# vita-epfl/trajnetplusplusbaselines

Measured on NVIDIA H100. Metric: pedestrian-steps/sec, higher is better.
Workload: dtype f32

## Files before the change

trajnetplusplusbaselines_b200/csrc/capi.cu:

```cuda
#include <algorithm>
#include <cstdio>
#include <cstdlib>
#include <cstring>
#include <new>

#include "common.cuh"

namespace tb2 {

static thread_local std::string g_error;
std::atomic<uint64_t> g_launch_count{0};

void set_error(const std::string& msg) { g_error = msg; }

struct ProfRec { const char* name; cudaEvent_t a, b; };
static bool g_profiling = false;
static std::vector<ProfRec> g_prof;

KernelTimer::KernelTimer(const char* name, cudaStream_t s) : slot(-1), st(s) {
    if (!g_profiling) return;
    ProfRec r;
    r.name = name;
    if (cudaEventCreate(&r.a) != cudaSuccess || cudaEventCreate(&r.b) != cudaSuccess) return;
    cudaEventRecord(r.a, st);
// ... 211 lines not shown
                TB2_REQUIRE(m->mlp_dims[i] >= 1, "MLP width");
            }
            m->pool_out = m->n_mlp == 0 ? m->mlp_dims[0] : c.out_dim;
            break;
        case TB2_POOL_NN_LSTM:
            TB2_REQUIRE(c.mlp_dim_hidden >= 1 && c.mlp_dim_hidden <= 512 && c.out_dim <= 1024 && c.mlp_dim_vel != 0,
                        "nearest-neighbour LSTM pooling needs 1 <= hidden_dim <= 512, out_dim <= 1024 and velocities");
            [[fallthrough]];
        case TB2_POOL_NN_MLP:
            TB2_REQUIRE(c.n >= 1 && c.n <= 32 && c.mlp_dim_spatial >= 1 && c.out_dim == c.n * c.mlp_dim_spatial,
                        "nearest-neighbour pooling needs 1 <= n <= 32 and out_dim == n * mlp_dim_spatial");
            m->pool_out = c.out_dim;
            break;
        case TB2_POOL_TRAJECTRON:
            TB2_REQUIRE(c.mlp_dim_hidden >= 1 && c.mlp_dim_hidden <= 512 && c.out_dim >= 1 && c.out_dim <= 1024,
                        "Trajectron pooling needs 1 <= hidden_dim <= 512 and out_dim <= 1024");
            m->pool_out = c.out_dim;
            break;
        case TB2_POOL_ATTN_MLP:
            TB2_REQUIRE(c.mlp_dim_spatial >= 1 && c.mlp_dim_vel >= 0 && c.mlp_dim_hidden >= 0 && c.out_dim >= 1 &&
                            c.mlp_dim_spatial + c.mlp_dim_vel + c.mlp_dim_hidden <= 128,
                        "attention pooling needs mlp_dim <= 128 (kernel specialisation)");
            m->pool_out = c.out_dim;
            break;
        case TB2_POOL_HIDDEN_MLP:
            TB2_REQUIRE(c.mlp_dim_spatial >= 1 && c.mlp_dim_vel >= 0 && c.mlp_dim_hidden >= 0 && c.out_dim >= 1 &&
                            c.mlp_dim_spatial + c.mlp_dim_vel + c.mlp_dim_hidden <= 4096,
                        "hidden-state MLP pooling widths");
            m->pool_out = c.out_dim;
            break;
    }
    TB2_REQUIRE(c.pool_to_input || m->pool_out == m->H, "pool_to_input=0 needs out_dim == hidden_dim");
    m->P = c.pool_to_input ? m->pool_out : 0;
    return TB2_OK;
}

static int alloc_buffers(tb2_lstm* m) {
    const tb2_lstm_config& c = m->cfg;
    int rc;
#define ALLOC(ptr, count) if ((rc = dev_alloc(m->owned, (void**)&(ptr), (size_t)(count) * sizeof(float)))) return rc
    ALLOC(m->We, (m->E - 2) * 2);
    ALLOC(m->be, m->E - 2);
    ALLOC(m->Wn, 5 * m->H);
    ALLOC(m->bn, 5);
    for (int ph = 0; ph < 2; ++ph) {
        ALLOC(m->WgT[ph], (size_t)m->K_gate_pad * 4 * m->H);
        ALLOC(m->bg[ph], 4 * m->H);
    }
    const bool no_tc = m->tc_disabled;
    if (!no_tc && gates_tc_supported(m)) {
        const size_t half = ((size_t)4 * m->H * m->K_gate + 1) / 2;
        for (int ph = 0; ph < 2; ++ph) {
            float *hi, *lo;
            ALLOC(hi, half);
            ALLOC(lo, half);
            m->Wg_hi[ph] = hi;
            m->Wg_lo[ph] = lo;
        }
    }
    const size_t Hp = (size_t)c.mlp_dim_hidden, D = (size_t)(c.mlp_dim_spatial + c.mlp_dim_vel + c.mlp_dim_hidden);
    auto encoder_lstm = [&]() {
        ALLOC(m->pl_WihT, (size_t)c.out_dim * 4 * Hp);
        ALLOC(m->pl_WhhT, Hp * 4 * Hp);
        ALLOC(m->pl_b, 4 * Hp);
        ALLOC(m->mp_WoT, Hp * (size_t)c.out_dim);
        ALLOC(m->mp_bo, c.out_dim);
        return TB2_OK;
    };
    switch (c.pool_type) {
        case TB2_POOL_NONE:
            break;
        case TB2_POOL_SOCIAL:
            ALLOC(m->WencT, m->H * m->C);
            ALLOC(m->benc, m->C);
            [[fallthrough]];
        case TB2_POOL_OCCUPANCY:
        case TB2_POOL_DIRECTIONAL:
            if (m->n_mlp == 0) break;
            ALLOC(m->Wt1, (size_t)m->cells * m->C * m->mlp_dims[1]);
            ALLOC(m->base1, m->mlp_dims[1]);
            if (c.pool_type == TB2_POOL_SOCIAL && m->C == 16 && !no_tc) {
                const size_t half = ((size_t)m->cells * 16 * m->mlp_dims[1] + 1) / 2;
                float *hi, *lo;
                ALLOC(hi, 2 * half);
                ALLOC(lo, 4);
                m->Wt1_hi = hi;
                m->Wt1_lo = lo;
            }
            for (int layer = 1; layer < m->n_mlp; ++layer) {
                ALLOC(m->WT[layer], (size_t)m->mlp_dims[layer] * m->mlp_dims[layer + 1]);
                ALLOC(m->bl[layer], m->mlp_dims[layer + 1]);
                if (layer == 1 && !no_tc && dense_tc_supported(m->mlp_dims[1], m->mlp_dims[2])) {
                    const size_t half = ((size_t)m->mlp_dims[1] * m->mlp_dims[2] + 1) / 2;
                    float *hi, *lo;
                    ALLOC(hi, half);
                    ALLOC(lo, half);
                    m->W_hi[1] = hi;
                    m->W_lo[1] = lo;
                }
            }
            break;
        case TB2_POOL_NN_LSTM:
            if ((rc = encoder_lstm())) return rc;
            [[fallthrough]];
        case TB2_POOL_NN_MLP:
            ALLOC(m->mp_Ws, c.mlp_dim_spatial * 4);
            ALLOC(m->mp_bs, c.mlp_dim_spatial);
            break;
        case TB2_POOL_TRAJECTRON:
            ALLOC(m->mp_Ws, (size_t)c.out_dim * 8);
            ALLOC(m->mp_bs, c.out_dim);
            if ((rc = encoder_lstm())) return rc;
            break;
        case TB2_POOL_ATTN_MLP:
            ALLOC(m->at_AqT, D * D);
            ALLOC(m->at_Ak, D * D);
            ALLOC(m->at_AvT, D * D);
            ALLOC(m->at_bqkv, 3 * D);
            ALLOC(m->at_WoT, D * D);
            ALLOC(m->at_bo, D);
            [[fallthrough]];
        case TB2_POOL_HIDDEN_MLP:
            ALLOC(m->mp_Ws, c.mlp_dim_spatial * 2);
            ALLOC(m->mp_bs, c.mlp_dim_spatial);
            ALLOC(m->mp_Wv, std::max(c.mlp_dim_vel, 1) * 2);
            ALLOC(m->mp_bv, std::max(c.mlp_dim_vel, 1));
            ALLOC(m->mp_WhT, (size_t)m->H * std::max(c.mlp_dim_hidden, 1));
            ALLOC(m->mp_bh, std::max(c.mlp_dim_hidden, 1));
            ALLOC(m->mp_WoT, D * c.out_dim);
            ALLOC(m->mp_bo, c.out_dim);
            break;
    }
#undef ALLOC
    return TB2_OK;
}

int tb2_lstm_create(const tb2_lstm_config* cfg, tb2_lstm** out) {
    TB2_REQUIRE(cfg && out, "null argument");
    *out = nullptr;
    if (!hidden_dim_supported(cfg->hidden_dim)) {
        set_error(kHiddenDimMessage);
        return TB2_ERR_UNSUPPORTED;
    }
    TB2_REQUIRE(cfg->embedding_dim >= 4 && cfg->embedding_dim <= 1024, "embedding_dim out of range");
    TB2_REQUIRE(cfg->pool_type >= TB2_POOL_NONE && cfg->pool_type <= TB2_POOL_TRAJECTRON, "bad pool_type");
    tb2_lstm* m = new (std::nothrow) tb2_lstm();
    TB2_REQUIRE(m, "out of host memory");
    m->cfg = *cfg;
    m->H = cfg->hidden_dim;
    m->E = cfg->embedding_dim;
    m->tc_disabled = tensor_cores_disabled();
    int rc = configure_pool(*cfg, m);
    if (rc == TB2_OK) {
        m->K_gate = m->E + m->P + m->H;
        m->K_gate_pad = (m->K_gate + kGateBK - 1) / kGateBK * kGateBK;
        rc = alloc_buffers(m);
    }
    if (rc != TB2_OK) {
        tb2_lstm_destroy(m);
        return rc;
    }
    *out = m;
    return TB2_OK;
}

int tb2_lstm_destroy(tb2_lstm* m) {
    if (!m) return TB2_OK;
// ... 336 lines not shown
```

trajnetplusplusbaselines_b200/csrc/common.cuh:

```cuda
#pragma once
#include <cuda_runtime.h>
#include <stdint.h>
#include <stddef.h>
#include <atomic>
#include <string>
#include <vector>

#include "trajnet_b200.h"

namespace tb2 {

void set_error(const std::string& msg);
extern std::atomic<uint64_t> g_launch_count;

#define TB2_CHECK_CUDA(expr)                                                              \
    do {                                                                                  \
        cudaError_t _e = (expr);                                                          \
        if (_e != cudaSuccess) {                                                          \
            ::tb2::set_error(std::string(#expr) + ": " + cudaGetErrorString(_e));         \
            return TB2_ERR_CUDA;                                                          \
        }                                                                                 \
    } while (0)

#define TB2_REQUIRE(cond, msg)                                                            \
// ... 7 lines not shown
#define TB2_LAUNCH_CHECK()                                                                \
    do {                                                                                  \
        ::tb2::g_launch_count.fetch_add(1, std::memory_order_relaxed);                    \
        TB2_CHECK_CUDA(cudaGetLastError());                                               \
    } while (0)

#ifdef __CUDACC__
__device__ __forceinline__ void grid_dep_wait() { asm volatile("griddepcontrol.wait;" ::: "memory"); }
__device__ __forceinline__ void grid_dep_launch() { asm volatile("griddepcontrol.launch_dependents;" ::: "memory"); }

__device__ __forceinline__ void mma_bf16_16816(float (&d)[4], const uint32_t (&a)[4], uint32_t b0, uint32_t b1) {
    asm volatile(
        "mma.sync.aligned.m16n8k16.row.col.f32.bf16.bf16.f32 {%0, %1, %2, %3}, {%4, %5, %6, %7}, {%8, %9}, "
        "{%0, %1, %2, %3};"
        : "+f"(d[0]), "+f"(d[1]), "+f"(d[2]), "+f"(d[3])
        : "r"(a[0]), "r"(a[1]), "r"(a[2]), "r"(a[3]), "r"(b0), "r"(b1));
}

template <typename... KArgs, typename... Args>
inline cudaError_t launch_pdl(void (*kernel)(KArgs...), dim3 grid, dim3 block, size_t smem, cudaStream_t st,
                              Args&&... args) {
    cudaLaunchConfig_t cfg = {};
    cfg.gridDim = grid;
    cfg.blockDim = block;
    cfg.dynamicSmemBytes = smem;
    cfg.stream = st;
    cudaLaunchAttribute attr[1];
    attr[0].id = cudaLaunchAttributeProgrammaticStreamSerialization;
    attr[0].val.programmaticStreamSerializationAllowed = 1;
    cfg.attrs = attr;
    cfg.numAttrs = 1;
    return cudaLaunchKernelEx(&cfg, kernel, static_cast<KArgs>(args)...);
}

template <typename... KArgs, typename... Args>
inline cudaError_t launch_pdl_cluster(void (*kernel)(KArgs...), dim3 grid, dim3 block, size_t smem, cudaStream_t st,
                                      unsigned cluster_x, Args&&... args) {
    cudaLaunchConfig_t cfg = {};
    cfg.gridDim = grid;
    cfg.blockDim = block;
    cfg.dynamicSmemBytes = smem;
    cfg.stream = st;
    cudaLaunchAttribute attr[2];
    attr[0].id = cudaLaunchAttributeProgrammaticStreamSerialization;
    attr[0].val.programmaticStreamSerializationAllowed = 1;
    attr[1].id = cudaLaunchAttributeClusterDimension;
    attr[1].val.clusterDim.x = cluster_x;
    attr[1].val.clusterDim.y = 1;
    attr[1].val.clusterDim.z = 1;
    cfg.attrs = attr;
    cfg.numAttrs = 2;
    return cudaLaunchKernelEx(&cfg, kernel, static_cast<KArgs>(args)...);
}
#endif

struct DynSmemConfig {
    size_t bytes[64];
    template <typename K>
    cudaError_t ensure(K kernel, size_t smem, size_t preset = 0) {
        int dev = 0;
        cudaError_t e = cudaGetDevice(&dev);
        if (e != cudaSuccess) return e;
        size_t& have = bytes[dev & 63];
        if (have < preset) have = preset;
        if (smem <= have) return cudaSuccess;
        e = cudaFuncSetAttribute(kernel, cudaFuncAttributeMaxDynamicSharedMemorySize, (int)smem);
        if (e == cudaSuccess) have = smem;
        return e;
    }
};

struct KernelTimer {
    KernelTimer(const char* name, cudaStream_t st);
    ~KernelTimer();
    int slot;
    cudaStream_t st;
};

constexpr int kMaxMlpLayers = 3;
constexpr int kMaxHidden = 256;
inline bool hidden_dim_supported(int H) { return H >= 32 && H <= kMaxHidden && H % 32 == 0; }
constexpr const char* kHiddenDimMessage = "hidden_dim must be a multiple of 32 from 32 to 256 (32, 64, 96, ..., 256)";
constexpr int kGateBK = 16;

}

struct tb2_lstm {
    tb2_lstm_config cfg = {};
    int H = 0, E = 0, C = 0, cells = 0, n_mlp = 0;
    int P = 0;
    int pool_out = 0;
    int mlp_dims[tb2::kMaxMlpLayers + 1] = {};
    int K_gate = 0, K_gate_pad = 0;
    bool weights_set = false;
    bool tc_disabled = false;
    float* We = nullptr;
    float* be = nullptr;
    float* WgT[2] = {};
    float* bg[2] = {};
    float* Wn = nullptr;
    float* bn = nullptr;
    float* WencT = nullptr;
    float* benc = nullptr;
    float* Wt1 = nullptr;
    float* base1 = nullptr;
    void* Wt1_hi = nullptr;
    void* Wt1_lo = nullptr;
    float* WT[tb2::kMaxMlpLayers] = {};
    float* bl[tb2::kMaxMlpLayers] = {};
    void* W_hi[tb2::kMaxMlpLayers] = {};
    void* W_lo[tb2::kMaxMlpLayers] = {};
    std::vector<cudaEvent_t> step_events;
    float *mp_Ws = nullptr, *mp_bs = nullptr, *mp_Wv = nullptr, *mp_bv = nullptr, *mp_WhT = nullptr, *mp_bh = nullptr,
          *mp_WoT = nullptr, *mp_bo = nullptr;
    float *at_AqT = nullptr, *at_Ak = nullptr, *at_AvT = nullptr, *at_bqkv = nullptr, *at_WoT = nullptr, *at_bo = nullptr;
    float *pl_WihT = nullptr, *pl_WhhT = nullptr, *pl_b = nullptr;
    void* Wg_hi[2] = {};
    void* Wg_lo[2] = {};
    std::vector<void*> owned;
};

struct tb2_layout {
    int B, M, n_max;
    int pad_to_max = 1;
    std::vector<int> scene_off_host;
    int* scene_off;
    int* row_scene;
    int group_cap[2];
    int num_groups[2];
    int* group_off[2];
    std::vector<void*> owned;
};

namespace tb2 {

struct Workspace {
    float* obs1;
    float* obs2;
    float* lat;
    int* win_count;
    uint32_t* win_ent;
    float* win_val;
    int* pair_cell;
    uint8_t* pair_flag;
    float* act[2];
    float* act2;
    float* pooled;
    void* emb_hi;
    void* emb_lo;
    void* pool_hi;
    void* pool_lo;
    void* hs_hi[2];
    void* hs_lo[2];
    size_t bytes;
    int write_pairs;
    float* pool_feat;
    float* pool_h;
    float* pool_c;
    float* scene_sum;
};

struct TrainCache {
    float* lat;
    int* win_count;
    uint32_t* win_ent;
    int* pair_cell;
// ... 50 lines not shown
```

trajnetplusplusbaselines_b200/csrc/pool.cu:

```cuda
#include <cuda_bf16.h>
#include <math_constants.h>
#include <algorithm>

#include "common.cuh"

namespace tb2 {

__global__ void resolve_obs_kernel(const float2* __restrict__ base, const float2* __restrict__ pred,
                                   const int* __restrict__ row_scene,
                                   const int* __restrict__ scene_off, float2* __restrict__ out, int M) {
    grid_dep_wait();
    grid_dep_launch();
    int m = blockIdx.x * blockDim.x + threadIdx.x;
    if (m >= M) return;
    bool primary = (scene_off[row_scene[m]] == m);
    out[m] = primary ? pred[m] : base[m];
}

int launch_resolve_obs(const tb2_layout* l, const float* base, const float* pred, float* out,
                       cudaStream_t st) {
    int threads = 256, blocks = (l->M + threads - 1) / threads;
    {
        KernelTimer kt("resolve_obs", st);
        launch_pdl(resolve_obs_kernel, dim3(blocks), dim3(threads), 0, st, (const float2*)base, (const float2*)pred,
                   (const int*)l->row_scene, (const int*)l->scene_off, (float2*)out, l->M);
    }
    TB2_LAUNCH_CHECK();
    return TB2_OK;
}

constexpr int kPrepMaxThreads = 640;
static int prep_threads(int n_max) { return 32 * std::min(std::max(n_max, 8), kPrepMaxThreads / 32); }
constexpr int kMaxSceneForPrep = 256;

struct PrepParams {
    const float2* obs1;
    const float2* obs2;
    const float* hidden;
    const int* scene_off;
    const float* WencT;
    const float* benc;
    float* lat;
    int* win_count;
    uint32_t* win_ent;
    float* win_val;
    int* pair_cell;
    uint8_t* pair_flag;
    const float* We;
    const float* be;
    __nv_bfloat16* emb_hi;
    __nv_bfloat16* emb_lo;
    int E;
    int n_max, H, C, n, pool_type, front, skip_masked, write_pairs, pad_to_max;
    float side, width;
};

__device__ __forceinline__ void cp_async16(void* smem, const void* gmem) {
    asm volatile("cp.async.cg.shared.global [%0], [%1], 16;" ::"r"((uint32_t)__cvta_generic_to_shared(smem)), "l"(gmem) : "memory");
}
__device__ __forceinline__ void cp_async_commit() { asm volatile("cp.async.commit_group;" ::: "memory"); }
__device__ __forceinline__ void cp_async_wait_all() { asm volatile("cp.async.wait_group 0;" ::: "memory"); }

__device__ __forceinline__ float nan_to_num_f(float x) {
    if (isnan(x)) return 0.f;
    if (isinf(x)) return x > 0 ? 3.402823466e+38f : -3.402823466e+38f;
    return x;
}

__global__ void __launch_bounds__(kPrepMaxThreads, 2) pool_prepare_kernel(PrepParams p) {
    const int kPrepThreads = (int)blockDim.x, kPrepWarps = kPrepThreads >> 5;
    extern __shared__ __align__(16) float smem_prep[];
    const int scene = blockIdx.x;
    const int row0 = p.scene_off[scene];
    const int n_s = p.scene_off[scene + 1] - row0;
    const int nm1 = p.n_max - 1;
    float2* pos = reinterpret_cast<float2*>(smem_prep);
    float2* vel = pos + n_s;
    int* cellrow = reinterpret_cast<int*>(vel + n_s);
    float* Ws = reinterpret_cast<float*>(cellrow + ((kPrepWarps * (nm1 > 0 ? nm1 : 1) + 3) & ~3));
    float* hs = Ws + (p.H + 8) * p.C;
    const int tid = threadIdx.x, lane = tid & 31, warp = tid >> 5;
    const bool social = p.pool_type == TB2_POOL_SOCIAL;
    const bool fast_lat = social && p.C == 16 && p.H == 128;
    if (fast_lat) {
        for (int idx = tid; idx < 128 * 4; idx += kPrepThreads) {
            const int k = idx >> 2, q4 = idx & 3;
            cp_async16(Ws + (k >> 4) * 272 + (k & 15) * 16 + q4 * 4, p.WencT + k * 16 + q4 * 4);
        }
    } else if (social) {
        for (int idx = tid; idx < p.H * p.C; idx += kPrepThreads) {
            const int k = idx / p.C, c = idx - k * p.C;
            Ws[c * (p.H + 4) + k] = p.WencT[idx];
        }
    }
    grid_dep_wait();
    grid_dep_launch();

    if (fast_lat) {
        const float* hsrc = p.hidden + (size_t)row0 * 128;
        for (int idx = tid; idx < n_s * 32; idx += kPrepThreads) cp_async16(hs + idx * 4, hsrc + idx * 4);
    }
    cp_async_commit();
    for (int j = tid; j < n_s; j += kPrepThreads) {
        float2 a = p.obs1[row0 + j], b = p.obs2[row0 + j];
        vel[j] = make_float2(b.x - a.x, b.y - a.y);
        if (isnan(b.x) || isnan(b.y)) b = make_float2(-500.f, -500.f);
        pos[j] = b;
    }
    if (social && !fast_lat) {
        const float4* hsrc = reinterpret_cast<const float4*>(p.hidden + (size_t)row0 * p.H);
        float4* hdst = reinterpret_cast<float4*>(hs);
        for (int idx = tid; idx < n_s * p.H / 4; idx += kPrepThreads) {
            float4 v = hsrc[idx];
            v.x = nan_to_num_f(v.x); v.y = nan_to_num_f(v.y); v.z = nan_to_num_f(v.z); v.w = nan_to_num_f(v.w);
            hdst[idx] = v;
        }
    }
    cp_async_wait_all();
    __syncthreads();
    if (p.emb_hi != nullptr) {
        const int e_shift = (p.E & (p.E - 1)) == 0 ? 31 - __clz(p.E) : -1;
        for (int idx = tid; idx < n_s * p.E; idx += kPrepThreads) {
            const int j = e_shift >= 0 ? idx >> e_shift : idx / p.E, k = idx - j * p.E;
            const float2 v = vel[j];
            float e = 0.f;
            if (k < p.E - 2 && !isnan(v.x))
                e = fmaxf(fmaf(p.We[2 * k + 1], v.y * 4.0f, fmaf(p.We[2 * k], v.x * 4.0f, p.be[k])), 0.f);
            const __nv_bfloat16 h = __float2bfloat16_rn(e);
            p.emb_hi[(size_t)(row0 + j) * p.E + k] = h;
            p.emb_lo[(size_t)(row0 + j) * p.E + k] = __float2bfloat16_rn(e - __bfloat162float(h));
        }
    }
    if (fast_lat) {
        const int c4 = lane & 3, kq = lane >> 2;
        const float4* wp = reinterpret_cast<const float4*>(Ws + kq * 272) + c4;
        const float4 bc = *reinterpret_cast<const float4*>(p.benc + c4 * 4);
        for (int j = warp; j < n_s; j += kPrepWarps) {
            const float4* hp = reinterpret_cast<const float4*>(hs + j * 128 + kq * 16);
            float4 acc = make_float4(0.f, 0.f, 0.f, 0.f);
#pragma unroll
            for (int q = 0; q < 4; ++q) {
// ... 284 lines not shown
        int incl = sum;
        for (int d = 1; d < 32; d <<= 1) {
            int v = __shfl_up_sync(0xffffffffu, incl, d);
            if (tid >= d) incl += v;
        }
        int run = incl - sum;
        for (int c = lo; c < hi; ++c) {
            int cnt = cursor[c];
            start[c] = run;
            cursor[c] = run;
            run += cnt;
        }
        if (tid == 31) start[bins] = incl;
    }
    __syncthreads();
    for (int idx = tid; idx < total; idx += kL1Threads) {
        int r = idx / p.nm1, k = idx - r * p.nm1;
        if (k < cnt_s[r]) {
            size_t g = (size_t)(row0 + r) * p.nm1 + k;
            uint32_t ent = raw[idx];
            int pos = atomicAdd(&cursor[(ent >> 16) * 2 + (r & 1)], 1);
            entP[pos] = (uint16_t)r;
            if (SOCIAL) {
                const int j = (int)(ent & 0xffff);
                entS[pos] = (uint16_t)(j == 0xffff ? p.cap : sbase[r] + j);
            } else {
#pragma unroll
                for (int c = 0; c < C; ++c) entV[(size_t)pos * C + c] = p.win_val[g * 2 + c] - p.constant;
            }
        }
    }
    __syncthreads();

    float w[C], wn[C];
    const float* wcol = p.Wt + col;
#pragma unroll
    for (int c = 0; c < C; ++c) w[c] = col_ok ? wcol[(size_t)c * p.OUT] : 0.f;
    for (int cell = 0; cell < p.cells; ++cell) {
        if (cell + 1 < p.cells) {
#pragma unroll
            for (int c = 0; c < C; ++c)
                wn[c] = col_ok ? wcol[((size_t)(cell + 1) * C + c) * p.OUT] : 0.f;
        }
        const int e0 = start[cell * 2 + half], e1 = start[cell * 2 + half + 1];
        for (int e = e0; e < e1; ++e) {
            const int r = entP[e];
            float a = acc[r * kL1Cols + colc];
            if (SOCIAL) {
                const float4* lv = reinterpret_cast<const float4*>(latS + (size_t)entS[e] * C);
#pragma unroll
                for (int c4 = 0; c4 < C / 4; ++c4) {
                    float4 v = lv[c4];
                    a = fmaf(v.x, w[c4 * 4 + 0], a);
                    a = fmaf(v.y, w[c4 * 4 + 1], a);
                    a = fmaf(v.z, w[c4 * 4 + 2], a);
                    a = fmaf(v.w, w[c4 * 4 + 3], a);
                }
            } else {
#pragma unroll
                for (int c = 0; c < C; ++c) a = fmaf(entV[(size_t)e * C + c], w[c], a);
            }
            acc[r * kL1Cols + colc] = a;
        }
#pragma unroll
        for (int c = 0; c < C; ++c) w[c] = wn[c];
    }
    __syncthreads();
    if (col_ok) {
        for (int r = half; r < P; r += 2) {
            float v = acc[r * kL1Cols + colc];
            if (p.relu) v = fmaxf(v, 0.f);
            const size_t o = (size_t)(row0 + r) * p.OUT + col;
            if (p.out_hi) {
                const __nv_bfloat16 h = __float2bfloat16_rn(v);
                p.out_hi[o] = h;
                p.out_lo[o] = __float2bfloat16_rn(v - __bfloat162float(h));
            } else {
                p.out[o] = v;
            }
        }
    }
}

constexpr int kMmaAccStride = kL1Cols + 16;

#ifndef TB2_L1_ABLATE
#define TB2_L1_ABLATE 0
#endif

__device__ __forceinline__ int kperm16(int k) { return 4 * ((k & 7) >> 1) + 2 * (k >> 3) + (k & 1); }

struct L1MmaParams {
    const int* group_off;
    const int* scene_off;
    const int* win_count;
    const uint32_t* win_ent;
    const float* lat;
    const float* benc;
    const __nv_bfloat16* Wt_hi;
    const __nv_bfloat16* Wt_lo;
    const float* base;
    float* out;
    __nv_bfloat16* out_hi;
    __nv_bfloat16* out_lo;
    int OUT, cells, nm1, cap, relu;
    float constant;
};

constexpr int kMmaThreads = 512;
constexpr int kMmaDepth = 8;
constexpr int kMmaMaxCap = 254;

__host__ __device__ inline size_t l1_mma_max_tiles(int cap, int cells, int nm1) { return ((size_t)cap * nm1 + (size_t)15 * cells) / 16; }

__host__ __device__ inline size_t l1_mma_slots(size_t max_tiles) { return 16 * max_tiles + 16 * kMmaDepth; }

__global__ void __launch_bounds__(kMmaThreads, 1) sparse_layer1_mma_kernel(L1MmaParams p) {
    extern __shared__ __align__(16) unsigned char smem_l1m[];
    const int tid = threadIdx.x, warp = tid >> 5, lane = tid & 31;
    const int g = lane >> 2, t = lane & 3;
    const int s0 = p.group_off[blockIdx.x], s1 = p.group_off[blockIdx.x + 1];
    const int row0 = p.scene_off[s0];
    const int P = p.scene_off[s1] - row0;
    const int chunk0 = blockIdx.y * kL1Cols;
    const size_t max_tiles = l1_mma_max_tiles(p.cap, p.cells, p.nm1);

    float* acc = reinterpret_cast<float*>(smem_l1m);
    __nv_bfloat16* lat = reinterpret_cast<__nv_bfloat16*>(acc + (size_t)p.cap * kMmaAccStride);
    int* start = reinterpret_cast<int*>(lat + (size_t)(p.cap + 2) * 32);
    int* cursor = start + p.cells + 1;
    uint16_t* tcell = reinterpret_cast<uint16_t*>(cursor + p.cells);
    uint16_t* ent = tcell + ((max_tiles + 1) & ~(size_t)1);
    uint32_t* raw = reinterpret_cast<uint32_t*>(ent + l1_mma_slots(max_tiles));
    int* cnt_s = reinterpret_cast<int*>(raw + (size_t)p.cap * p.nm1);
    int* sbase = cnt_s + p.cap;

    for (int c = tid; c < p.cells; c += kMmaThreads) cursor[c] = 0;
    for (int sb = s0 + warp; sb < s1; sb += kMmaThreads / 32) {
        const int a = p.scene_off[sb] - row0, b = p.scene_off[sb + 1] - row0;
        for (int r = a + lane; r < b; r += 32) sbase[r] = a;
    }
    {
        const uint32_t pad = ((uint32_t)(p.cap + 1) << 8) | 0xffu;
        uint32_t* ent2 = reinterpret_cast<uint32_t*>(ent);
        for (int idx = tid; idx < (int)(l1_mma_slots(max_tiles) / 2); idx += kMmaThreads) ent2[idx] = pad | (pad << 16);
    }
    const int ew = (tid >> 2) & 15, et = tid & 3;
    const int ecol = chunk0 + ew * 16 + 2 * et;
    {
        float4 b4;
        b4.x = ecol < p.OUT ? p.base[ecol] : 0.f;
        b4.y = ecol + 1 < p.OUT ? p.base[ecol + 1] : 0.f;
        b4.z = ecol + 8 < p.OUT ? p.base[ecol + 8] : 0.f;
        b4.w = ecol + 9 < p.OUT ? p.base[ecol + 9] : 0.f;
        for (int r = tid >> 6; r < P; r += kMmaThreads / 64)
            *reinterpret_cast<float4*>(acc + r * kMmaAccStride + ew * 16 + 4 * et) = b4;
    }
    grid_dep_wait();
    grid_dep_launch();
    for (int r = tid; r < P; r += kMmaThreads) cnt_s[r] = p.win_count[row0 + r];
    {
        const uint32_t* src = p.win_ent + (size_t)row0 * p.nm1;
        for (int idx = tid; idx < P * p.nm1; idx += kMmaThreads) raw[idx] = src[idx];
    }
    for (int idx = tid; idx < (P + 2) * 16; idx += kMmaThreads) {
        const int r = idx >> 4, k = idx & 15;
        float v = 0.f;
        if (r < P) v = p.lat[(size_t)(row0 + r) * 16 + k] - p.constant;
        else if (r == P) v = p.benc[k] - p.constant;
        const __nv_bfloat16 h = __float2bfloat16_rn(v);
        const int kp = kperm16(k);
        const int dst = (r < P ? r : p.cap + (r - P)) * 32 + (kp >> 2) * 8 + (kp & 3);
        lat[dst] = h;
        lat[dst + 4] = __float2bfloat16_rn(v - __bfloat162float(h));
    }
    __syncthreads();
    const int total = P * p.nm1;
    for (int idx = tid; idx < total; idx += kMmaThreads) {
        int r = idx / p.nm1, k = idx - r * p.nm1;
        if (k < cnt_s[r]) atomicAdd(&cursor[raw[idx] >> 16], 1);
    }
    __syncthreads();
    if (tid < 32) {
        int per = (p.cells + 31) / 32;
        int lo = tid * per, hi = min(lo + per, p.cells);
        int sum = 0;
        for (int c = lo; c < hi; ++c) sum += (cursor[c] + 15) & ~15;
        int incl = sum;
        for (int d = 1; d < 32; d <<= 1) {
            int v = __shfl_up_sync(0xffffffffu, incl, d);
            if (tid >= d) incl += v;
        }
        int run = incl - sum;
        for (int c = lo; c < hi; ++c) {
            const int padded = (cursor[c] + 15) & ~15;
            start[c] = run;
            cursor[c] = run;
            for (int k = run >> 4; k < (run + padded) >> 4; ++k) tcell[k] = (uint16_t)c;
            run += padded;
        }
        if (tid == 31) start[p.cells] = incl;
    }
    __syncthreads();
    for (int idx = tid; idx < total; idx += kMmaThreads) {
        int r = idx / p.nm1, k = idx - r * p.nm1;
        if (k < cnt_s[r]) {
            const uint32_t e = raw[idx];
            const int pos = atomicAdd(&cursor[e >> 16], 1);
            const int j = (int)(e & 0xffff);
            const uint32_t lrow = (uint32_t)(j == 0xffff ? p.cap : sbase[r] + j);
            ent[(pos & ~15) + 2 * (pos & 7) + ((pos >> 3) & 1)] = (uint16_t)((lrow << 8) | (uint32_t)r);
        }
    }
    __syncthreads();

    const int tiles = start[p.cells] >> 4;
    const int ncol0 = chunk0 + warp * 16 + g;
    const uint32_t cell_stride = (uint32_t)p.OUT * 32;
    const __nv_bfloat16* wh = p.Wt_hi + (size_t)ncol0 * 32 + 8 * t;
    bool okc[2];
#pragma unroll
    for (int j = 0; j < 2; ++j) okc[j] = ncol0 + 8 * j < p.OUT;
    struct BFrag { uint2 h[2], l[2]; };
    auto load_b = [&](int cell) -> BFrag {
#if TB2_L1_ABLATE == 2
        cell = 0;
#endif
        const __nv_bfloat16* w = wh + (uint32_t)cell * cell_stride;
        BFrag f;
#pragma unroll
        for (int j = 0; j < 2; ++j) {
            const uint4 v = okc[j] ? __ldcg(reinterpret_cast<const uint4*>(w + j * 8 * 32))
                                   : make_uint4(0u, 0u, 0u, 0u);
            f.h[j] = make_uint2(v.x, v.y);
            f.l[j] = make_uint2(v.z, v.w);
        }
        return f;
    };
    struct Tile { uint32_t e; uint4 a0, a1; };
    const uint4* latT = reinterpret_cast<const uint4*>(lat) + t;
    const uint32_t* ent2 = reinterpret_cast<const uint32_t*>(ent);
    auto fetch = [&](int k) -> Tile {
        Tile f;
        f.e = ent2[8 * k + g];
        f.a0 = latT[((f.e >> 8) & 0xffu) * 4];
        f.a1 = latT[(f.e >> 24) * 4];
        return f;
    };
    float* accw = acc + warp * 16 + 4 * t;
    BFrag b[kMmaDepth];
#pragma unroll
    for (int i = 0; i < kMmaDepth; ++i) b[i] = load_b(i < tiles ? tcell[i] : 0);
    Tile cur = fetch(0);
#if TB2_L1_ABLATE == 1
    float4 s0a = make_float4(0.f, 0.f, 0.f, 0.f), s1a = s0a;
#endif
    for (int k0 = 0; k0 < tiles; k0 += kMmaDepth) {
#pragma unroll
        for (int i = 0; i < kMmaDepth; ++i) {
            const int k = k0 + i;
            const uint32_t r0 = cur.e & 0xffu, r1 = (cur.e >> 16) & 0xffu;
            const bool v0 = r0 != 0xffu, v1 = r1 != 0xffu;
            float4* q0 = reinterpret_cast<float4*>(accw + r0 * kMmaAccStride);
            float4* q1 = reinterpret_cast<float4*>(accw + r1 * kMmaAccStride);
            float4 u0, u1;
#if TB2_L1_ABLATE == 1
            u0 = s0a; u1 = s1a;
#else
            if (v0) u0 = *q0;
            if (v1) u1 = *q1;
#endif
            const Tile nxt = fetch(k + 1);
            const uint32_t ah[4] = {cur.a0.x, cur.a1.x, cur.a0.y, cur.a1.y};
            const uint32_t al[4] = {cur.a0.z, cur.a1.z, cur.a0.w, cur.a1.w};
            float d[2][4];
#pragma unroll
            for (int j = 0; j < 2; ++j) {
#if TB2_L1_ABLATE == 3
#pragma unroll
                for (int x = 0; x < 4; ++x)
                    d[j][x] = __uint_as_float((ah[x] ^ b[i].h[j].x ^ b[i].l[j].y) + (al[x] ^ b[i].h[j].y ^ b[i].l[j].x));
#else
                d[j][0] = d[j][1] = d[j][2] = d[j][3] = 0.f;
                mma_bf16_16816(d[j], ah, b[i].h[j].x, b[i].h[j].y);
                mma_bf16_16816(d[j], ah, b[i].l[j].x, b[i].l[j].y);
                mma_bf16_16816(d[j], al, b[i].h[j].x, b[i].h[j].y);
#endif
            }
            u0 = make_float4(u0.x + d[0][0], u0.y + d[0][1], u0.z + d[1][0], u0.w + d[1][1]);
            u1 = make_float4(u1.x + d[0][2], u1.y + d[0][3], u1.z + d[1][2], u1.w + d[1][3]);
#if TB2_L1_ABLATE == 1
            if (v0) s0a = u0;
            if (v1) s1a = u1;
#else
            if (v0) *q0 = u0;
            if (v1) *q1 = u1;
#endif
            if (k + kMmaDepth < tiles) b[i] = load_b(tcell[k + kMmaDepth]);
            cur = nxt;
        }
    }
#if TB2_L1_ABLATE == 1
    if (P > 0) {
        *reinterpret_cast<float4*>(accw + (g % P) * kMmaAccStride) = s0a;
        __syncwarp();
        *reinterpret_cast<float4*>(accw + ((g + 8) % P) * kMmaAccStride) = s1a;
    }
#endif
    __syncthreads();
    const bool odd = et & 1;
    const int ocol = odd ? ecol + 6 : ecol;
    const bool vec = (p.OUT & 3) == 0;
    for (int r = tid >> 6; r < P; r += kMmaThreads / 64) {
        const float4 a = *reinterpret_cast<const float4*>(acc + r * kMmaAccStride + ew * 16 + 4 * et);
        const float sx = __shfl_xor_sync(0xffffffffu, odd ? a.x : a.z, 1);
        const float sy = __shfl_xor_sync(0xffffffffu, odd ? a.y : a.w, 1);
        float v[4] = {odd ? sx : a.x, odd ? sy : a.y, odd ? a.z : sx, odd ? a.w : sy};
        if (p.relu) {
#pragma unroll
            for (int x = 0; x < 4; ++x) v[x] = fmaxf(v[x], 0.f);
        }
        const size_t o = (size_t)(row0 + r) * p.OUT + ocol;
        if (p.out_hi) {
            __align__(8) __nv_bfloat16 h[4], l[4];
#pragma unroll
            for (int x = 0; x < 4; ++x) {
                h[x] = __float2bfloat16_rn(v[x]);
                l[x] = __float2bfloat16_rn(v[x] - __bfloat162float(h[x]));
            }
            if (vec) {
                if (ocol < p.OUT) {
                    *reinterpret_cast<uint2*>(p.out_hi + o) = *reinterpret_cast<const uint2*>(h);
                    *reinterpret_cast<uint2*>(p.out_lo + o) = *reinterpret_cast<const uint2*>(l);
                }
            } else {
#pragma unroll
                for (int x = 0; x < 4; ++x)
                    if (ocol + x < p.OUT) { p.out_hi[o + x] = h[x]; p.out_lo[o + x] = l[x]; }
            }
        } else if (vec) {
            if (ocol < p.OUT) *reinterpret_cast<float4*>(p.out + o) = make_float4(v[0], v[1], v[2], v[3]);
        } else {
#pragma unroll
            for (int x = 0; x < 4; ++x)
                if (ocol + x < p.OUT) p.out[o + x] = v[x];
        }
    }
}

static size_t l1_mma_smem_bytes(int cap, int cells, int nm1) {
    const size_t tiles = l1_mma_max_tiles(cap, cells, nm1);
    size_t b = (size_t)cap * kMmaAccStride * sizeof(float);
    b += (size_t)(cap + 2) * 32 * sizeof(__nv_bfloat16);
    b += (size_t)(2 * cells + 1) * sizeof(int);
    b += ((tiles + 1) & ~(size_t)1) * sizeof(uint16_t);
    b += l1_mma_slots(tiles) * sizeof(uint16_t);
    b += (size_t)cap * nm1 * sizeof(uint32_t);
    b += (size_t)cap * 2 * sizeof(int);
    return b + 16;
}

static DynSmemConfig l1_mma_smem_config;

int layer1_mma_info(int cap, int cells, int nm1, int* chunk_cols, int* threads, int* ctas_per_sm) {
    const size_t sm = l1_mma_smem_bytes(cap, cells, nm1);
    TB2_REQUIRE(sm <= 227 * 1024 && cap <= kMmaMaxCap, "scene group does not fit in shared memory (scene too large)");
    TB2_CHECK_CUDA(l1_mma_smem_config.ensure(sparse_layer1_mma_kernel, sm));
    TB2_CHECK_CUDA(cudaOccupancyMaxActiveBlocksPerMultiprocessor(ctas_per_sm, sparse_layer1_mma_kernel, kMmaThreads, sm));
    *chunk_cols = kL1Cols;
    *threads = kMmaThreads;
    return TB2_OK;
}

__global__ void repack_layer1_mma_kernel(const float* __restrict__ W1, __nv_bfloat16* __restrict__ hi,
                                         __nv_bfloat16* __restrict__ lo, int OUT, int cells) {
    size_t total = (size_t)cells * OUT * 16;
    for (size_t idx = (size_t)blockIdx.x * blockDim.x + threadIdx.x; idx < total;
         idx += (size_t)gridDim.x * blockDim.x) {
        const int c = (int)(idx & 15);
        const size_t co = idx >> 4;
        const int o = (int)(co % OUT), cell = (int)(co / OUT);
        const float v = W1[(size_t)o * 16 * cells + (size_t)c * cells + cell];
        const __nv_bfloat16 h = __float2bfloat16_rn(v);
        const int kp = kperm16(c);
        const size_t dst = (co << 5) + (size_t)(kp >> 2) * 8 + (kp & 3);
        hi[dst] = h;
        hi[dst + 4] = __float2bfloat16_rn(v - __bfloat162float(h));
        (void)lo;
    }
}

int launch_repack_layer1_mma(const float* W1, void* hi, void* lo, int OUT, int cells, cudaStream_t st) {
    repack_layer1_mma_kernel<<<1024, 256, 0, st>>>(W1, (__nv_bfloat16*)hi, (__nv_bfloat16*)lo, OUT, cells);
    TB2_LAUNCH_CHECK();
    return TB2_OK;
}

static size_t l1_smem_bytes(int cap, int C, bool social, int cells, int nm1) {
    size_t b = (size_t)cap * kL1Cols * sizeof(float);
    if (social) b += (size_t)(cap + 1) * C * sizeof(float);
    b += (size_t)(4 * cells + 1) * sizeof(int);
    size_t ents = ((size_t)cap * nm1 * 2 * sizeof(uint16_t) + 15) & ~(size_t)15;
    b += ents;
    if (!social) b += (size_t)cap * nm1 * C * sizeof(float);
    b += (size_t)cap * nm1 * sizeof(uint32_t) + (size_t)cap * 2 * sizeof(int);
    return b + 16;
}

struct RowsParams {
    const int* win_count;
    const uint32_t* win_ent;
    const float* win_val;
    const float* Wt;
    const float* base;
    float* out;
    __nv_bfloat16* out_hi;
    __nv_bfloat16* out_lo;
    int M, OUT, cells, C, nm1, CH, rows_per_cta, relu;
    float constant;
};

constexpr int kRowsThreads = 1024;

__global__ void __launch_bounds__(kRowsThreads, 1) pool_rows_kernel(RowsParams p) {
    extern __shared__ __align__(16) unsigned char smem_rows[];
    float* Ws = reinterpret_cast<float*>(smem_rows);
    const int KW = p.cells * p.C;
    int* cnt_s = reinterpret_cast<int*>(Ws + (size_t)KW * p.CH);
    uint32_t* ent_s = reinterpret_cast<uint32_t*>(cnt_s + p.rows_per_cta);
    float* val_s = reinterpret_cast<float*>(ent_s + (size_t)p.rows_per_cta * p.nm1);
    const int tid = threadIdx.x;
    grid_dep_wait();
    grid_dep_launch();
    const int col0 = blockIdx.y * p.CH;
    const int r0 = blockIdx.x * p.rows_per_cta;
    const int nrows = min(p.rows_per_cta, p.M - r0);
    if (nrows <= 0) return;
    const int cw = min(p.CH, p.OUT - col0);
    if ((p.OUT & 3) == 0 && (cw & 3) == 0) {
        const int q = cw >> 2;
        for (int idx = tid; idx < KW * q; idx += kRowsThreads) {
            const int k = idx / q, c4 = idx - k * q;
            *reinterpret_cast<float4*>(Ws + (size_t)k * p.CH + c4 * 4) =
                *reinterpret_cast<const float4*>(p.Wt + (size_t)k * p.OUT + col0 + c4 * 4);
        }
    } else {
        for (int idx = tid; idx < KW * cw; idx += kRowsThreads) {
            const int k = idx / cw, c = idx - k * cw;
            Ws[(size_t)k * p.CH + c] = p.Wt[(size_t)k * p.OUT + col0 + c];
        }
    }
    for (int r = tid; r < nrows; r += kRowsThreads) cnt_s[r] = p.win_count[r0 + r];
    {
        const uint32_t* esrc = p.win_ent + (size_t)r0 * p.nm1;
        for (int idx = tid; idx < nrows * p.nm1; idx += kRowsThreads) ent_s[idx] = esrc[idx];
        const float* vsrc = p.win_val + (size_t)r0 * p.nm1 * 2;
        for (int idx = tid; idx < nrows * p.nm1 * 2; idx += kRowsThreads) val_s[idx] = vsrc[idx] - p.constant;
    }
    __syncthreads();
    const int lanes = kRowsThreads / p.CH;
    const int colc = tid % p.CH, lane = tid / p.CH;
    const int col = col0 + colc;
    if (col >= p.OUT) return;
    const float b = p.base[col];
    for (int r = lane; r < nrows; r += lanes) {
        float acc = b;
        const int cnt = cnt_s[r];
        const uint32_t* er = ent_s + (size_t)r * p.nm1;
        const float* vr = val_s + (size_t)r * p.nm1 * 2;
        for (int e = 0; e < cnt; ++e) {
            const float* w = Ws + (size_t)(er[e] >> 16) * p.C * p.CH + colc;
            acc = fmaf(w[0], vr[2 * e], acc);
            if (p.C == 2) acc = fmaf(w[p.CH], vr[2 * e + 1], acc);
        }
        if (p.relu) acc = fmaxf(acc, 0.f);
        const size_t o = (size_t)(r0 + r) * p.OUT + col;
        if (p.out_hi) {
// ... 179 lines not shown
```

Measured before the change: 29.01 million.

## Widen layer-1 MMA warp tiles to 32 columns and software-pipeline the tile loop

The sparse layer-1 MMA kernel now runs 256 threads, and each warp covers 32 output columns (four n-fragments) instead of 16. Each gathered A tile is therefore reused across twice as many MMAs, and the per-column bounds checks are dropped by zero-padding the weight image past OUT. The tile loop is software-pipelined one tile further: the next tile's MMA is issued before the current result is accumulated, and entry and cell indices are prefetched. The preamble uses cp.async for counts and entries and vectorized float4 latent loads, and the accumulator row padding is shrunk. In exchange, register pressure goes up and there are half as many warps to hide latency, and the shared-memory accumulator stride change may introduce bank conflicts.

```diff
diff --git a/trajnetplusplusbaselines_b200/csrc/capi.cu b/trajnetplusplusbaselines_b200/csrc/capi.cu
--- a/trajnetplusplusbaselines_b200/csrc/capi.cu
+++ b/trajnetplusplusbaselines_b200/csrc/capi.cu
@@ -317,7 +317,7 @@
             if (c.pool_type == TB2_POOL_SOCIAL && m->C == 16 && !no_tc) {
                 const size_t half = ((size_t)m->cells * 16 * m->mlp_dims[1] + 1) / 2;
                 float *hi, *lo;
-                ALLOC(hi, 2 * half);
+                ALLOC(hi, 2 * half + (size_t)kLayer1MmaTailCols * 16);
                 ALLOC(lo, 4);
                 m->Wt1_hi = hi;
                 m->Wt1_lo = lo;
diff --git a/trajnetplusplusbaselines_b200/csrc/common.cuh b/trajnetplusplusbaselines_b200/csrc/common.cuh
--- a/trajnetplusplusbaselines_b200/csrc/common.cuh
+++ b/trajnetplusplusbaselines_b200/csrc/common.cuh
@@ -113,6 +113,7 @@
 inline bool hidden_dim_supported(int H) { return H >= 32 && H <= kMaxHidden && H % 32 == 0; }
 constexpr const char* kHiddenDimMessage = "hidden_dim must be a multiple of 32 from 32 to 256 (32, 64, 96, ..., 256)";
 constexpr int kGateBK = 16;
+constexpr int kLayer1MmaTailCols = 256;
 
 }
 
diff --git a/trajnetplusplusbaselines_b200/csrc/pool.cu b/trajnetplusplusbaselines_b200/csrc/pool.cu
--- a/trajnetplusplusbaselines_b200/csrc/pool.cu
+++ b/trajnetplusplusbaselines_b200/csrc/pool.cu
@@ -57,6 +57,9 @@
 
 __device__ __forceinline__ void cp_async16(void* smem, const void* gmem) {
     asm volatile("cp.async.cg.shared.global [%0], [%1], 16;" ::"r"((uint32_t)__cvta_generic_to_shared(smem)), "l"(gmem) : "memory");
+}
+__device__ __forceinline__ void cp_async4(void* smem, const void* gmem) {
+    asm volatile("cp.async.ca.shared.global [%0], [%1], 4;" ::"r"((uint32_t)__cvta_generic_to_shared(smem)), "l"(gmem) : "memory");
 }
 __device__ __forceinline__ void cp_async_commit() { asm volatile("cp.async.commit_group;" ::: "memory"); }
 __device__ __forceinline__ void cp_async_wait_all() { asm volatile("cp.async.wait_group 0;" ::: "memory"); }
@@ -507,7 +510,7 @@
     }
 }
 
-constexpr int kMmaAccStride = kL1Cols + 16;
+constexpr int kMmaAccStride = kL1Cols + 4;
 
 #ifndef TB2_L1_ABLATE
 #define TB2_L1_ABLATE 0
@@ -532,13 +535,17 @@
     float constant;
 };
 
-constexpr int kMmaThreads = 512;
+constexpr int kMmaThreads = 256;
 constexpr int kMmaDepth = 8;
 constexpr int kMmaMaxCap = 254;
 
 __host__ __device__ inline size_t l1_mma_max_tiles(int cap, int cells, int nm1) { return ((size_t)cap * nm1 + (size_t)15 * cells) / 16; }
 
-__host__ __device__ inline size_t l1_mma_slots(size_t max_tiles) { return 16 * max_tiles + 16 * kMmaDepth; }
+__host__ __device__ inline size_t l1_mma_slots(size_t max_tiles) { return 16 * max_tiles + 16 * (kMmaDepth + 2); }
+
+#if TB2_L1_ABLATE == 4
+constexpr size_t kMmaAblateSlab = (size_t)kL1Cols * 32 * sizeof(__nv_bfloat16);
+#endif
 
 __global__ void __launch_bounds__(kMmaThreads, 1) sparse_layer1_mma_kernel(L1MmaParams p) {
     extern __shared__ __align__(16) unsigned char smem_l1m[];
@@ -570,8 +577,9 @@
         uint32_t* ent2 = reinterpret_cast<uint32_t*>(ent);
         for (int idx = tid; idx < (int)(l1_mma_slots(max_tiles) / 2); idx += kMmaThreads) ent2[idx] = pad | (pad << 16);
     }
-    const int ew = (tid >> 2) & 15, et = tid & 3;
-    const int ecol = chunk0 + ew * 16 + 2 * et;
+    const int ew = (tid >> 3) & 7, eh = (tid >> 2) & 1, et = tid & 3;
+    const int ecol = chunk0 + ew * 32 + eh * 16 + 2 * et;
+    const int eword = ew * 32 + 8 * et + 4 * eh;
     {
         float4 b4;
         b4.x = ecol < p.OUT ? p.base[ecol] : 0.f;
@@ -579,26 +587,34 @@
         b4.z = ecol + 8 < p.OUT ? p.base[ecol + 8] : 0.f;
         b4.w = ecol + 9 < p.OUT ? p.base[ecol + 9] : 0.f;
         for (int r = tid >> 6; r < P; r += kMmaThreads / 64)
-            *reinterpret_cast<float4*>(acc + r * kMmaAccStride + ew * 16 + 4 * et) = b4;
+            *reinterpret_cast<float4*>(acc + r * kMmaAccStride + eword) = b4;
     }
     grid_dep_wait();
     grid_dep_launch();
-    for (int r = tid; r < P; r += kMmaThreads) cnt_s[r] = p.win_count[row0 + r];
+    for (int r = tid; r < P; r += kMmaThreads) cp_async4(cnt_s + r, p.win_count + row0 + r);
     {
         const uint32_t* src = p.win_ent + (size_t)row0 * p.nm1;
-        for (int idx = tid; idx < P * p.nm1; idx += kMmaThreads) raw[idx] = src[idx];
-    }
-    for (int idx = tid; idx < (P + 2) * 16; idx += kMmaThreads) {
-        const int r = idx >> 4, k = idx & 15;
-        float v = 0.f;
-        if (r < P) v = p.lat[(size_t)(row0 + r) * 16 + k] - p.constant;
-        else if (r == P) v = p.benc[k] - p.constant;
-        const __nv_bfloat16 h = __float2bfloat16_rn(v);
-        const int kp = kperm16(k);
-        const int dst = (r < P ? r : p.cap + (r - P)) * 32 + (kp >> 2) * 8 + (kp & 3);
-        lat[dst] = h;
-        lat[dst + 4] = __float2bfloat16_rn(v - __bfloat162float(h));
-    }
+        for (int idx = tid; idx < P * p.nm1; idx += kMmaThreads) cp_async4(raw + idx, src + idx);
+    }
+    cp_async_commit();
+    for (int idx = tid; idx < (P + 2) * 4; idx += kMmaThreads) {
+        const int r = idx >> 2, k0 = (idx & 3) * 4;
+        float4 v4 = make_float4(0.f, 0.f, 0.f, 0.f);
+        if (r < P) v4 = *reinterpret_cast<const float4*>(p.lat + (size_t)(row0 + r) * 16 + k0);
+        else if (r == P) v4 = *reinterpret_cast<const float4*>(p.benc + k0);
+        const float vk[4] = {v4.x, v4.y, v4.z, v4.w};
+        const int row = r < P ? r : p.cap + (r - P);
+#pragma unroll
+        for (int i = 0; i < 4; ++i) {
+            const float v = r <= P ? vk[i] - p.constant : 0.f;
+            const __nv_bfloat16 h = __float2bfloat16_rn(v);
+            const int kp = kperm16(k0 + i);
+            const int dst = row * 32 + (kp >> 2) * 8 + (kp & 3);
+            lat[dst] = h;
+            lat[dst + 4] = __float2bfloat16_rn(v - __bfloat162float(h));
+        }
+    }
+    cp_async_wait_all();
     __syncthreads();
     const int total = P * p.nm1;
     for (int idx = tid; idx < total; idx += kMmaThreads) {
@@ -640,13 +656,18 @@
     __syncthreads();
 
     const int tiles = start[p.cells] >> 4;
-    const int ncol0 = chunk0 + warp * 16 + g;
+    const int ncol0 = chunk0 + warp * 32 + g;
     const uint32_t cell_stride = (uint32_t)p.OUT * 32;
     const __nv_bfloat16* wh = p.Wt_hi + (size_t)ncol0 * 32 + 8 * t;
-    bool okc[2];
-#pragma unroll
-    for (int j = 0; j < 2; ++j) okc[j] = ncol0 + 8 * j < p.OUT;
-    struct BFrag { uint2 h[2], l[2]; };
+#if TB2_L1_ABLATE == 4
+    uint4* wslab = reinterpret_cast<uint4*>((reinterpret_cast<uintptr_t>(sbase + p.cap) + 15) & ~(uintptr_t)15) + warp * 128;
+    for (int i = lane; i < 128; i += 32) {
+        const int c = chunk0 + warp * 32 + (i >> 2);
+        wslab[i] = c < p.OUT ? __ldcg(reinterpret_cast<const uint4*>(p.Wt_hi + (size_t)c * 32) + (i & 3)) : make_uint4(0u, 0u, 0u, 0u);
+    }
+    __syncwarp();
+#endif
+    struct BFrag { uint2 h[4], l[4]; };
     auto load_b = [&](int cell) -> BFrag {
 #if TB2_L1_ABLATE == 2
         cell = 0;
@@ -654,9 +675,13 @@
         const __nv_bfloat16* w = wh + (uint32_t)cell * cell_stride;
         BFrag f;
 #pragma unroll
-        for (int j = 0; j < 2; ++j) {
-            const uint4 v = okc[j] ? __ldcg(reinterpret_cast<const uint4*>(w + j * 8 * 32))
-                                   : make_uint4(0u, 0u, 0u, 0u);
+        for (int j = 0; j < 4; ++j) {
+#if TB2_L1_ABLATE == 4
+            (void)w;
+            const uint4 v = wslab[(8 * j + g) * 4 + t];
+#else
+            const uint4 v = __ldcg(reinterpret_cast<const uint4*>(w + j * 8 * 32));
+#endif
             f.h[j] = make_uint2(v.x, v.y);
             f.l[j] = make_uint2(v.z, v.w);
         }
@@ -665,20 +690,41 @@
     struct Tile { uint32_t e; uint4 a0, a1; };
     const uint4* latT = reinterpret_cast<const uint4*>(lat) + t;
     const uint32_t* ent2 = reinterpret_cast<const uint32_t*>(ent);
-    auto fetch = [&](int k) -> Tile {
+    auto a_rows = [&](uint32_t e) -> Tile {
         Tile f;
-        f.e = ent2[8 * k + g];
-        f.a0 = latT[((f.e >> 8) & 0xffu) * 4];
-        f.a1 = latT[(f.e >> 24) * 4];
+        f.e = e;
+        f.a0 = latT[((e >> 8) & 0xffu) * 4];
+        f.a1 = latT[(e >> 24) * 4];
         return f;
     };
-    float* accw = acc + warp * 16 + 4 * t;
+    auto tile_mma = [&](const Tile& a, const BFrag& bf, float (&d)[4][4]) {
+        const uint32_t ah[4] = {a.a0.x, a.a1.x, a.a0.y, a.a1.y};
+        const uint32_t al[4] = {a.a0.z, a.a1.z, a.a0.w, a.a1.w};
+#pragma unroll
+        for (int j = 0; j < 4; ++j) {
+#if TB2_L1_ABLATE == 3
+#pragma unroll
+            for (int x = 0; x < 4; ++x)
+                d[j][x] = __uint_as_float((ah[x] ^ bf.h[j].x ^ bf.l[j].y) + (al[x] ^ bf.h[j].y ^ bf.l[j].x));
+#else
+            d[j][0] = d[j][1] = d[j][2] = d[j][3] = 0.f;
+            mma_bf16_16816(d[j], ah, bf.h[j].x, bf.h[j].y);
+            mma_bf16_16816(d[j], ah, bf.l[j].x, bf.l[j].y);
+            mma_bf16_16816(d[j], al, bf.h[j].x, bf.h[j].y);
+#endif
+        }
+    };
+    float* accw = acc + warp * 32 + 8 * t;
     BFrag b[kMmaDepth];
 #pragma unroll
     for (int i = 0; i < kMmaDepth; ++i) b[i] = load_b(i < tiles ? tcell[i] : 0);
-    Tile cur = fetch(0);
+    Tile cur = a_rows(ent2[g]), nxt = a_rows(ent2[8 + g]);
+    uint32_t e2 = ent2[16 + g];
+    int cell_ahead = kMmaDepth < tiles ? tcell[kMmaDepth] : 0;
+    float d[4][4];
+    tile_mma(cur, b[0], d);
 #if TB2_L1_ABLATE == 1
-    float4 s0a = make_float4(0.f, 0.f, 0.f, 0.f), s1a = s0a;
+    float4 s0a = make_float4(0.f, 0.f, 0.f, 0.f), s0b = s0a, s1a = s0a, s1b = s0a;
 #endif
     for (int k0 = 0; k0 < tiles; k0 += kMmaDepth) {
 #pragma unroll
@@ -688,48 +734,45 @@
             const bool v0 = r0 != 0xffu, v1 = r1 != 0xffu;
             float4* q0 = reinterpret_cast<float4*>(accw + r0 * kMmaAccStride);
             float4* q1 = reinterpret_cast<float4*>(accw + r1 * kMmaAccStride);
-            float4 u0, u1;
+            float4 u0a, u0b, u1a, u1b;
 #if TB2_L1_ABLATE == 1
-            u0 = s0a; u1 = s1a;
+            u0a = s0a; u0b = s0b; u1a = s1a; u1b = s1b;
 #else
-            if (v0) u0 = *q0;
-            if (v1) u1 = *q1;
+            if (v0) { u0a = q0[0]; u0b = q0[1]; }
+            if (v1) { u1a = q1[0]; u1b = q1[1]; }
 #endif
-            const Tile nxt = fetch(k + 1);
-            const uint32_t ah[4] = {cur.a0.x, cur.a1.x, cur.a0.y, cur.a1.y};
-            const uint32_t al[4] = {cur.a0.z, cur.a1.z, cur.a0.w, cur.a1.w};
-            float d[2][4];
-#pragma unroll
-            for (int j = 0; j < 2; ++j) {
-#if TB2_L1_ABLATE == 3
-#pragma unroll
-                for (int x = 0; x < 4; ++x)
-                    d[j][x] = __uint_as_float((ah[x] ^ b[i].h[j].x ^ b[i].l[j].y) + (al[x] ^ b[i].h[j].y ^ b[i].l[j].x));
+            float dn[4][4];
+            tile_mma(nxt, b[(i + 1) % kMmaDepth], dn);
+            const Tile nn = a_rows(e2);
+            e2 = ent2[8 * (k + 3) + g];
+            u0a = make_float4(u0a.x + d[0][0], u0a.y + d[0][1], u0a.z + d[1][0], u0a.w + d[1][1]);
+            u0b = make_float4(u0b.x + d[2][0], u0b.y + d[2][1], u0b.z + d[3][0], u0b.w + d[3][1]);
+            u1a = make_float4(u1a.x + d[0][2], u1a.y + d[0][3], u1a.z + d[1][2], u1a.w + d[1][3]);
+            u1b = make_float4(u1b.x + d[2][2], u1b.y + d[2][3], u1b.z + d[3][2], u1b.w + d[3][3]);
+#if TB2_L1_ABLATE == 1
+            if (v0) { s0a = u0a; s0b = u0b; }
+            if (v1) { s1a = u1a; s1b = u1b; }
 #else
-                d[j][0] = d[j][1] = d[j][2] = d[j][3] = 0.f;
-                mma_bf16_16816(d[j], ah, b[i].h[j].x, b[i].h[j].y);
-                mma_bf16_16816(d[j], ah, b[i].l[j].x, b[i].l[j].y);
-                mma_bf16_16816(d[j], al, b[i].h[j].x, b[i].h[j].y);
+            if (v0) { q0[0] = u0a; q0[1] = u0b; }
+            if (v1) { q1[0] = u1a; q1[1] = u1b; }
 #endif
-            }
-            u0 = make_float4(u0.x + d[0][0], u0.y + d[0][1], u0.z + d[1][0], u0.w + d[1][1]);
-            u1 = make_float4(u1.x + d[0][2], u1.y + d[0][3], u1.z + d[1][2], u1.w + d[1][3]);
-#if TB2_L1_ABLATE == 1
-            if (v0) s0a = u0;
-            if (v1) s1a = u1;
-#else
-            if (v0) *q0 = u0;
-            if (v1) *q1 = u1;
-#endif
-            if (k + kMmaDepth < tiles) b[i] = load_b(tcell[k + kMmaDepth]);
+            if (k + kMmaDepth < tiles) b[i] = load_b(cell_ahead);
+            cell_ahead = k + kMmaDepth + 1 < tiles ? tcell[k + kMmaDepth + 1] : 0;
+#pragma unroll
+            for (int j = 0; j < 4; ++j)
+#pragma unroll
+                for (int x = 0; x < 4; ++x) d[j][x] = dn[j][x];
             cur = nxt;
+            nxt = nn;
         }
     }
 #if TB2_L1_ABLATE == 1
     if (P > 0) {
-        *reinterpret_cast<float4*>(accw + (g % P) * kMmaAccStride) = s0a;
+        float4* q0 = reinterpret_cast<float4*>(accw + (g % P) * kMmaAccStride);
+        q0[0] = s0a; q0[1] = s0b;
         __syncwarp();
-        *reinterpret_cast<float4*>(accw + ((g + 8) % P) * kMmaAccStride) = s1a;
+        float4* q1 = reinterpret_cast<float4*>(accw + ((g + 8) % P) * kMmaAccStride);
+        q1[0] = s1a; q1[1] = s1b;
     }
 #endif
     __syncthreads();
@@ -737,7 +780,7 @@
     const int ocol = odd ? ecol + 6 : ecol;
     const bool vec = (p.OUT & 3) == 0;
     for (int r = tid >> 6; r < P; r += kMmaThreads / 64) {
-        const float4 a = *reinterpret_cast<const float4*>(acc + r * kMmaAccStride + ew * 16 + 4 * et);
+        const float4 a = *reinterpret_cast<const float4*>(acc + r * kMmaAccStride + eword);
         const float sx = __shfl_xor_sync(0xffffffffu, odd ? a.x : a.z, 1);
         const float sy = __shfl_xor_sync(0xffffffffu, odd ? a.y : a.w, 1);
         float v[4] = {odd ? sx : a.x, odd ? sy : a.y, odd ? a.z : sx, odd ? a.w : sy};
@@ -782,6 +825,9 @@
     b += l1_mma_slots(tiles) * sizeof(uint16_t);
     b += (size_t)cap * nm1 * sizeof(uint32_t);
     b += (size_t)cap * 2 * sizeof(int);
+#if TB2_L1_ABLATE == 4
+    b += 16 + kMmaAblateSlab;
+#endif
     return b + 16;
 }
 
@@ -816,8 +862,11 @@
 }
 
 int launch_repack_layer1_mma(const float* W1, void* hi, void* lo, int OUT, int cells, cudaStream_t st) {
+    static_assert(kLayer1MmaTailCols >= kL1Cols, "a chunk's columns past OUT must stay inside the weight image");
     repack_layer1_mma_kernel<<<1024, 256, 0, st>>>(W1, (__nv_bfloat16*)hi, (__nv_bfloat16*)lo, OUT, cells);
     TB2_LAUNCH_CHECK();
+    TB2_CHECK_CUDA(cudaMemsetAsync((__nv_bfloat16*)hi + (size_t)cells * OUT * 32, 0,
+                                   (size_t)kLayer1MmaTailCols * 32 * sizeof(__nv_bfloat16), st));
     return TB2_OK;
 }
 
```

Result: faster. 31.33 million, median of 6 (+8.0%).
